# slp-rl/aero

Measured on AMD Instinct MI355X. Metric: real-time-factor (audio-sec/wall-sec), Aero.forward STFT+U-Net+iSTFT, 4->16kHz nfft=512 hop=64 batch=64 per GPU, higher is better.
Workload: dtype f16; 1 GPU; batch=64 synthetic 2s white-noise clips per GPU, 4->16 kHz, aero_4-16_512_64 (nfft=512 hop=64), random-init weights seed 2036, inference, inputs resident in HBM; global_batch=64, clip_samples=8000, frames=501, parallelism=clips sharded over 1 GPU(s), no data-path collective, precision=fp16 operands/storage, fp32 accumulate; STFT/iSTFT/statistics fp32

## Files before the change

aero_amd/_lib.py:

```python
import ctypes as C
import os

_HERE = os.path.dirname(os.path.abspath(__file__))
DEFAULT_LIB = os.path.join(_HERE, 'libaero_hip.so')

ACT_NONE, ACT_RELU, ACT_GELU, ACT_GLU, ACT_SNAKE = 0, 1, 2, 3, 4

i32, i64, vp, fp, dp = C.c_int32, C.c_int64, C.c_void_p, C.c_void_p, C.c_void_p


class ConvDesc(C.Structure):
    _fields_ = [('src0', vp), ('s0_b', i64), ('s0_f', i64), ('s0_t', i64), ('C0', i32),
                ('src1', vp), ('s1_b', i64), ('s1_f', i64), ('s1_t', i64), ('C1', i32),
                ('weight', vp), ('bias', fp),
                ('dst', vp), ('d_b', i64), ('d_f', i64), ('d_t', i64),
                ('dst_f32', i32), ('dst_f_off', i32), ('dst_F', i32),
                ('B', i32), ('Fin', i32), ('Fout', i32), ('T', i32), ('M', i32),
                ('transposed', i32), ('fstride', i32),
                ('ntaps', i32), ('df', i32 * 9), ('dt', i32 * 9),
                ('act', i32),
                ('res', vp), ('r_b', i64), ('r_f', i64), ('r_t', i64),
                ('post_add', fp), ('batch_scale', fp), ('batch_shift', fp),
                ('stats', dp), ('stat_count', C.c_double),
                ('stat_mode', i32), ('stat_G', i32), ('stat_per_row', i32), ('stat_eps', C.c_float),
# ... 88 lines not shown
                ('B', i32), ('F', i32), ('T', i32), ('C', i32)]


class FtbFirstDesc(C.Structure):
    _fields_ = [('xn', vp), ('u', vp), ('gate', vp), ('w2a', vp),
                ('p0', fp), ('p1', fp), ('pb', fp), ('rs', fp), ('a_re', fp), ('a_im', fp), ('bias', fp),
                ('dst', vp), ('B', i32), ('F', i32), ('T', i32), ('C', i32)]


class Enc0Desc(C.Structure):
    _fields_ = [('xn', vp), ('u', vp), ('g', vp), ('rs', fp), ('a_re', fp), ('a_im', fp), ('bias_f', fp),
                ('wc', vp), ('bias_c', fp), ('dst', vp),
                ('B', i32), ('F', i32), ('T', i32), ('C', i32), ('M', i32), ('Fo', i32), ('ktaps', i32), ('stride', i32),
                ('pad', i32), ('act', i32)]


class SeanetConvDesc(C.Structure):
    _fields_ = [('x', vp), ('wimg', vp), ('bias', fp), ('add', vp), ('y', vp),
                ('B', i32), ('Tin', i32), ('Cin', i32), ('Tq', i32), ('M', i32), ('K', i32), ('stride', i32), ('dil', i32), ('pad', i32),
                ('reflect', i32), ('ksteps', i32), ('R', i32), ('P', i32), ('Tout', i32), ('Cout', i32), ('act', i32), ('in_slope', C.c_float)]


class SeanetResDesc(C.Structure):
    _fields_ = [('x', vp), ('w1', vp), ('w2s', vp), ('b1', fp), ('b2s', fp), ('add', vp), ('y', vp),
                ('B', i32), ('T', i32), ('C', i32), ('d', i32), ('ks1', i32), ('ks2', i32), ('slope', C.c_float)]


DCONV_MAX_DEPTH = 4


class DconvLayer(C.Structure):
    _fields_ = [('w1', vp), ('w2', vp), ('consts', fp), ('snake_a', fp),
                ('dilation', i32), ('norm1', i32), ('norm2', i32), ('reserved', i32)]


class DconvDesc(C.Structure):
    _fields_ = [('x', vp), ('y', vp), ('R', i32), ('T', i32), ('C', i32), ('hidden', i32), ('depth', i32), ('act', i32),
                ('F', i32), ('eps', C.c_float), ('layer', DconvLayer * DCONV_MAX_DEPTH)]


class DconvRewriteDesc(C.Structure):
    _fields_ = [('dconv', DconvDesc), ('rw_w', vp), ('rw_bias', fp), ('post_add', fp),
                ('dst', vp), ('d_b', i64), ('d_f', i64), ('d_t', i64)]


_PROTOS = {
    'aero_version': (C.c_char_p, []),
    'aero_last_error': (C.c_char_p, []),
    'aero_last_kernel_name': (C.c_char_p, []),
    'aero_stft_fwd': (i32, [fp, i32, i32, i32, i32, i32, fp, i32, fp, i32, dp, i32, vp]),
    'aero_stft_dft_table_bytes': (i64, [i32]),
    'aero_stft_dft_table': (i32, [fp, i32, i32, vp, vp]),
    'aero_stft_dft_fwd': (i32, [fp, i32, i32, i32, i32, i32, i32, vp, fp, i32, dp, i32, vp]),
    'aero_stft_dft_norm_fwd': (i32, [fp, i32, i32, i32, i32, i32, i32, vp, i32, dp, i32, vp, fp, vp]),
    'aero_spec_normalize': (i32, [fp, i32, i64, dp, vp, fp, vp]),
    'aero_istft_fwd': (i32, [fp, i32, i32, i32, i32, i32, fp, fp, fp, i32, vp]),
    'aero_istft_pitch': (i32, [i32, i32, i32, C.POINTER(i32), C.POINTER(i32)]),
    'aero_istft_pitched_fwd': (i32, [fp, i32, i32, i32, i32, i32, i32, i32, fp, fp, fp, i32, vp]),
    'aero_conv_fwd': (i32, [C.POINTER(ConvDesc), vp]),
    'aero_split_finish': (i32, [fp, i32, fp, i32, vp, i64, i32, vp]),
    'aero_adam_step': (i32, [fp, fp, fp, fp, i64, C.c_float, C.c_float, C.c_float, C.c_float, i32, C.c_float, vp]),
    'aero_adam_step_dev': (i32, [fp, fp, fp, fp, i64, C.c_float, C.c_float, C.c_float, C.c_float, fp, C.c_float, vp]),
    'aero_conv_wgrad': (i32, [C.POINTER(WgradDesc), vp]),
    'aero_conv_wgrad_chunks': (i32, [i32, i32, i32, i32, i32]),
    'aero_norm_bwd_reduce': (i32, [C.POINTER(NormBwdDesc), vp]),
    'aero_norm_bwd_apply': (i32, [C.POINTER(NormBwdDesc), vp]),
    'aero_istft_bwd_prep': (i32, [fp, fp, fp, i32, i32, i32, i32, i32, vp]),
    'aero_istft_bwd_pack': (i32, [fp, fp, i32, i32, i32, i32, i32, vp]),
    'aero_conv_tile_m': (i32, [i32]),
    'aero_conv_ring_bm': (i32, [i32, i32]),
    'aero_convtr_tail_finish': (i32, [fp, fp, fp, fp, fp, fp, i32, i32, i32, i32, i32, vp]),
    'aero_convtr_tail_finish_pitched': (i32, [fp, fp, fp, fp, fp, fp, i32, i32, i32, i32, i32, i32, i32, vp]),
    'aero_conv_kernel_name': (i32, [C.POINTER(ConvDesc), C.c_char_p, i32]),
    'aero_norm_stats': (i32, [C.POINTER(NormDesc), vp]),
    'aero_norm_apply': (i32, [C.POINTER(NormDesc), vp]),
    'aero_gram_stats': (i32, [C.POINTER(GramDesc), vp]),
    'aero_lstm_fwd': (i32, [C.POINTER(LstmDesc), vp]),
    'aero_lstm_geometry': (i32, [i32, C.POINTER(i32), C.POINTER(i32)]),
    'aero_lstm_geometry_in': (i32, [i32, i32, C.POINTER(i32)]),
    'aero_localstate_fwd': (i32, [C.POINTER(AttnDesc), vp]),
    'aero_freqfc_fwd': (i32, [C.POINTER(FreqFcDesc), vp]),
    'aero_ftb_first_fwd': (i32, [C.POINTER(FtbFirstDesc), vp]),
    'aero_enc0_fwd': (i32, [C.POINTER(Enc0Desc), vp]),
    'aero_dconv_row_fwd': (i32, [C.POINTER(DconvDesc), vp]),
    'aero_dconv_row_fits': (i32, [i32, i32, i32, i32]),
    'aero_dconv_row_rewrite_fwd': (i32, [C.POINTER(DconvRewriteDesc), vp]),
    'aero_dconv_row_rewrite_fits': (i32, [i32, i32, i32, i32]),
    'aero_lstm_bwd': (i32, [C.POINTER(LstmBwdDesc), vp]),
    'aero_lstm_bwd_k4p': (i32, [i32]),
    'aero_localstate_bwd': (i32, [C.POINTER(AttnBwdDesc), vp]),
    'aero_freqfc_wgrad': (i32, [vp, vp, vp, fp, fp, i32, i32, i32, i32, i32, vp]),
    'aero_ftb_gate_bwd': (i32, [vp, vp, vp, vp, vp, vp, i32, i32, i32, i32, vp]),
    'aero_sum_bt': (i32, [vp, fp, i32, i32, i32, i32, C.c_float, vp]),
    'aero_frames_op': (i32, [vp, vp, i32, i32, i32, i32, i32, i32, i32, vp]),
    'aero_stft_loss_sums': (i32, [fp, fp, i64, C.c_float, dp, i32, dp, vp]),
    'aero_stft_loss_bwd': (i32, [fp, fp, i64, C.c_float, dp, C.c_float, C.c_float, fp, fp, vp]),
    'aero_irfft_frames': (i32, [fp, i32, i32, i32, i32, fp, fp, vp]),
    'aero_stft_adj_fold': (i32, [fp, fp, i32, i32, i32, i32, i32, i32, vp]),
    'aero_add_f16': (i32, [vp, vp, vp, i64, C.c_float, vp]),
    'aero_scale_cast': (i32, [fp, i32, i64, fp, vp, C.c_float, vp, fp, vp]),
    'aero_scale_f32': (i32, [fp, i64, fp, vp]),
    'aero_gather_pack': (i32, [vp, vp, i32, vp, vp, i64, i32, vp]),
    'aero_debug_probe': (i32, [vp, i32, i32, i32, vp, vp]),
    'aero_bn_running_update': (i32, [dp, i32, C.c_double, C.c_float, fp, fp, vp, vp]),
    'aero_gconv1d_mfma_ok': (i32, [i32, i32, i32, i32, i32, i32, i32]),
    'aero_weightnorm_fwd': (i32, [fp, fp, fp, i32, i32, vp]),
    'aero_weightnorm_bwd': (i32, [fp, i64, i64, i64, fp, fp, fp, fp, fp, fp, fp, fp, i32, i32, i32, i32, vp]),
    'aero_gconv1d_wgrad_slabs': (i32, [i32, i32, i32, i32, i32, i32, i32, i32, i32]),
    'aero_rescale_f16': (i32, [vp, fp, vp, fp, i64, vp, C.c_float, vp, fp, vp]),
    'aero_gconv1d_fwd': (i32, [C.POINTER(GconvDesc), vp]),
    'aero_pw_fwd': (i32, [C.POINTER(PwDesc), vp]),
    'aero_comm_unique_id': (i32, [vp]),
    'aero_comm_init': (i32, [i32, i32, vp, C.POINTER(vp)]),
    'aero_allreduce_f32': (i32, [vp, fp, i64, vp]),
    'aero_allgather': (i32, [vp, vp, vp, i64, vp]),
    'aero_comm_destroy': (i32, [vp]),
    'aero_stream_create': (i32, [i32, C.POINTER(C.c_uint32), i32, C.POINTER(vp)]),
    'aero_stream_destroy': (i32, [vp]),
    'aero_pw_rows': (i32, [i32, i32]),
    'aero_pw_ksteps': (i32, [i32]),
    'aero_squeeze_fwd': (i32, [vp, i64, i64, i64, vp, fp, vp, i32, i32, i32, i32, i32, i32, i32, vp]),
    'aero_leaky_relu': (i32, [vp, i64, C.c_float, vp]),
    'aero_avgpool1d': (i32, [vp, vp, i32, i32, vp]),
    'aero_loss_sum': (i32, [vp, vp, i64, C.c_float, i32, dp, i32, dp, C.c_double, vp]),
    'aero_gconv1d_bwd': (i32, [C.POINTER(GconvBwdDesc), vp]),
    'aero_loss_grad': (i32, [vp, vp, i64, C.c_float, C.c_float, i32, vp, fp, vp]),
    'aero_avgpool1d_bwd': (i32, [vp, vp, i32, i32, vp]),
    'aero_mpd_fold': (i32, [fp, i32, i32, i32, vp, vp]),
    'aero_mpd_unfold_add': (i32, [fp, i32, i32, i32, fp, vp]),
    'aero_mpd_conv0_fwd': (i32, [vp, fp, fp, vp, i32, i32, i32, i32, C.c_float, vp]),
    'aero_mpd_conv0_slabs': (i32, [i32, i32]),
    'aero_mpd_conv0_bwd': (i32, [vp, vp, fp, fp, fp, fp, i32, fp, fp, i32, i32, i32, i32, vp]),
    'aero_mpd_act': (i32, [vp, i32, i32, i32, i32, C.c_float, vp]),
    'aero_seanet_stats': (i32, [fp, i32, i32, C.c_float, fp, vp]),
    'aero_seanet_front': (i32, [fp, fp, fp, fp, i32, i32, i32, i32, i32, i32, i32, vp]),
    'aero_seanet_conv_in': (i32, [fp, fp, fp, vp, i32, i32, i32, vp]),
    'aero_seanet_conv': (i32, [C.POINTER(SeanetConvDesc), vp]),
    'aero_seanet_resblock': (i32, [C.POINTER(SeanetResDesc), vp]),
    'aero_seanet_conv_out': (i32, [vp, vp, fp, fp, fp, fp, i32, i32, i32, i32, C.c_float, vp]),
    'aero_segment_gather': (i32, [vp, i32, vp, vp, i32, vp, vp, i32, i32, fp, vp]),
    'aero_overlap_stitch': (i32, [fp, i32, fp, i32, fp, i32, i32, i64, i32, i32, i32, fp, i64, vp, vp]),
    'aero_wav_finalize': (i32, [fp, vp, i32, i64, fp, vp]),
}

EXPORTS = tuple(_PROTOS)


class AeroHipError(RuntimeError):
    pass


class Lib:

    def __init__(self, path):
        if not os.path.exists(path):
            raise ImportError(
                f'{path} not found: build the gfx950 kernels first (python -c "import __graft_entry__ as g; '
                f'g.build()").  aero_amd has no CPU or eager fallback.')
        self.path = path
        self.cdll = C.CDLL(path)
        for name, (res, args) in _PROTOS.items():
            try:
                fn = getattr(self.cdll, name)
            except AttributeError as e:
                raise ImportError(f'{path} does not export {name}') from e
            fn.restype = res
# ... 34 lines not shown
```

aero_amd/csrc/aero_hip.hip:

```cpp
#include "aero_common.h"
#ifdef AERO_PART
#define AERO_IN(p) (AERO_PART == (p))
#else
#define AERO_IN(p) 1
#endif
#if AERO_IN(0)
#include "k_attn.h"
#include "k_lstm.h"
#include "k_norm.h"
#include "k_gram.h"
#include "k_optim.h"
#endif
#if AERO_IN(1)
#include "k_stft.h"
#include "k_train.h"
#endif
#if AERO_IN(2)
#include "k_conv.h"
#endif
#if AERO_IN(6)
#include "k_conv_ring.h"
#endif
#if AERO_IN(7)
#include "k_pw.h"
// ... 371 lines not shown
}

int aero_scale_f32(float* x, int64_t n, const float* scale, void* stream) {
    const char* err = "";
    int rc = aero_scale_f32_launch(x, n, scale, (hipStream_t)stream, &err);
    return aero_finish(rc, err);
}

int aero_rescale_f16(const void* a, const float* sa, const void* b, const float* sb, int64_t n, void* amax, float target, void* out,
                     float* scale_out, void* stream) {
    const char* err = "";
    int rc = aero_rescale_f16_launch(a, sa, b, sb, n, (unsigned int*)amax, target, out, scale_out, (hipStream_t)stream, &err);
    return aero_finish(rc, err);
}

#endif

#if AERO_IN(2)

int aero_conv_fwd(const aero_conv_desc* d, void* stream) {
    const char* err = "";
    AeroConvK p;
    AeroConvPlan plan;
    int rc = aero_conv_check(d, &err);
    if (rc == AERO_OK) rc = aero_conv_plan(d, p, plan, &err);
    if (rc == AERO_OK) aero_conv_issue(plan, p, (hipStream_t)stream);
    return aero_finish(rc, err);
}

int aero_conv_tile_m(int32_t M) { return aero_conv_pick_bm(M, (M + 127) / 128 * 128); }

int aero_conv_kernel_name(const aero_conv_desc* d, char* name, int32_t cap) {
    if (!name || cap < 96) return aero_fail(AERO_ERR_ARG, "conv_kernel_name: buffer of >= 96 bytes required");
    const char* err = "";
    name[0] = 0;
    AeroConvK p;
    AeroConvPlan plan;
    int rc = aero_conv_check(d, &err);
    if (rc == AERO_OK) rc = aero_conv_plan(d, p, plan, &err);
    if (rc != AERO_OK) return aero_fail(rc, err);
    aero_conv_plan_name(plan, name);
    return AERO_OK;
}

int aero_split_finish(const float* acc, int32_t nsplit, const float* bias, int32_t act, void* dst, int64_t npos, int32_t M, void* stream) {
    const char* err = "";
    int rc = aero_split_finish_launch(acc, nsplit, bias, act, dst, npos, M, (hipStream_t)stream, &err);
    return aero_finish(rc, err);
}

#endif

#if AERO_IN(3)

int aero_freqfc_fwd(const aero_freqfc_desc* d, void* stream) {
    const char* err = "";
    int rc = aero_freqfc_launch(d, (hipStream_t)stream, &err);
    return aero_finish(rc, err);
}

int aero_dconv_row_fwd(const aero_dconv_desc* d, void* stream) {
    const char* err = "";
    int rc = aero_dconv_launch(d, nullptr, (hipStream_t)stream, &err);
    return aero_finish(rc, err);
}

int aero_dconv_row_fits(int T, int C, int hidden, int max_dilation) { return aero_dconv_row_fits_impl(T, C, hidden, max_dilation); }

int aero_dconv_row_rewrite_fwd(const aero_dconv_rewrite_desc* d, void* stream) {
    const char* err = "";
    if (!d) return aero_fail(AERO_ERR_ARG, "dconv rewrite: null descriptor");
    int rc = aero_dconv_launch(&d->dconv, d, (hipStream_t)stream, &err);
    return aero_finish(rc, err);
}

int aero_dconv_row_rewrite_fits(int T, int C, int hidden, int max_dilation) { return aero_dconv_row_fits_impl(T, C, hidden, max_dilation, true); }

int aero_enc0_fwd(const aero_enc0_desc* d, void* stream) {
    const char* err = "";
    int rc = aero_enc0_launch(d, (hipStream_t)stream, &err);
    return aero_finish(rc, err);
}

int aero_ftb_first_fwd(const aero_ftb_first_desc* d, void* stream) {
    const char* err = "";
    int rc = aero_ftb_first_launch(d, (hipStream_t)stream, &err);
    return aero_finish(rc, err);
}

#endif

#if AERO_IN(4)

int aero_conv_wgrad(const aero_wgrad_desc* d, void* stream) {
    const char* err = "";
    int rc = aero_conv_wgrad_launch(d, (hipStream_t)stream, &err);
    return aero_finish(rc, err);
}

int aero_conv_wgrad_chunks(int32_t M, int32_t C, int32_t ntaps, int32_t nrows, int32_t T) {
    if (M < 1 || C < 1 || ntaps < 1 || nrows < 1 || T < 1) return 1;
    bool big;
    int nchunk, SC;
    aero_wgrad_plan(M, C, ntaps, nrows, T, &big, &nchunk, &SC);
    return nchunk;
}

int aero_norm_bwd_reduce(const aero_norm_bwd_desc* d, void* stream) {
    const char* err = "";
    int rc = aero_norm_bwd_launch(d, 0, (hipStream_t)stream, &err);
    return aero_finish(rc, err);
}

int aero_norm_bwd_apply(const aero_norm_bwd_desc* d, void* stream) {
    const char* err = "";
    int rc = aero_norm_bwd_launch(d, 1, (hipStream_t)stream, &err);
    return aero_finish(rc, err);
}

int aero_istft_bwd_prep(const float* dy, const float* inv_env, float* s, int32_t nsig, int32_t L, int32_t Ls, int32_t off, int32_t env_off, void* stream) {
    const char* err = "";
    int rc = aero_istft_bwd_prep_launch(dy, inv_env, s, nsig, L, Ls, off, env_off, (hipStream_t)stream, &err);
    return aero_finish(rc, err);
}

int aero_istft_bwd_pack(const float* spec, float* dz, int32_t nsig, int32_t nbins, int32_t Tsrc, int32_t T, int32_t t_off, void* stream) {
    const char* err = "";
    int rc = aero_istft_bwd_pack_launch(spec, dz, nsig, nbins, Tsrc, T, t_off, (hipStream_t)stream, &err);
    return aero_finish(rc, err);
}

#endif

#if AERO_IN(4)

int aero_gconv1d_mfma_ok(int32_t Cin, int32_t Cout, int32_t groups, int32_t K, int32_t stride, int32_t pad, int32_t reflect) {
    return aero_gconv4_ok(Cin, Cout, groups, K, stride, pad, reflect);
}

int aero_gconv1d_wgrad_slabs(int32_t B, int32_t Tin, int32_t Cin, int32_t Cout, int32_t groups, int32_t K, int32_t stride, int32_t pad,
                             int32_t reflect) {
    if (B < 1 || Tin < 1) return 0;
    const bool c1 = aero_edge_c1_ok(Cin, Cout, groups, K, stride, pad);
    if (c1 || aero_edge_o1_ok(Cin, Cout, groups, K, stride, pad, reflect)) {
        int nb, per;
        aero_edge_wgrad_plan(c1, B, Tin, &nb, &per);
        return B * nb;
    }
    if (!aero_gconv4_ok(Cin, Cout, groups, K, stride, pad, reflect)) return 0;
    const int Tout = (Tin + 2 * pad - K) / stride + 1;
    if (Tout < 1) return 0;
    int ntile, tpc, nchunk;
    aero_gconv4_wgrad_plan(B, Tout, groups, &ntile, &tpc, &nchunk);
    return B * nchunk;
}

int aero_weightnorm_fwd(const float* v, const float* g, float* w, int32_t Cout, int32_t L, void* stream) {
    if (!v || !g || !w || Cout < 1 || L < 1) return aero_fail(AERO_ERR_ARG, "weightnorm_fwd: bad arguments");
    AERO_LAUNCH(aero_weightnorm_fwd_kernel, dim3((unsigned)Cout), dim3(256), (hipStream_t)stream, v, g, w, L);
    return aero_finish(AERO_OK, "");
}

int aero_weightnorm_bwd(const float* dw, int64_t so, int64_t sc, int64_t sk, const float* v, const float* g, const float* db, const float* inv_scale,
                        const float* gl, float* dg, float* dv, float* dbias, int32_t Cout, int32_t cig, int32_t K, int32_t accumulate, void* stream) {
    const char* err = "";
    int rc = aero_weightnorm_bwd_launch(dw, so, sc, sk, v, g, db, inv_scale, gl, dg, dv, dbias, Cout, cig, K, accumulate, (hipStream_t)stream, &err);
// ... 295 lines not shown
```

aero_amd/csrc/k_enc0.h:

```cpp
#pragma once
#include "aero_common.h"

static __device__ __forceinline__ h16x8 aero_splat8(h16 v) { return (h16x8){v, v, v, v, v, v, v, v}; }

struct AeroEnc0K {
    aero_enc0_desc d;
    int Cp, Mpad, Ktot;
};

template <int MFC, int KT, int ROWS>
__global__ __launch_bounds__(256, 2) void aero_enc0_kernel(AeroEnc0K p) {
    constexpr int BN = 128;
    constexpr int BMC = MFC * 16;
    constexpr int CS = BMC + 8;
    h16* Ws = (h16*)AERO_DYN_SMEM;
    const aero_enc0_desc& d = p.d;
    const int nrows = (ROWS - 1) * d.stride + d.ktaps;
    h16* Cs = Ws + d.ktaps * KT * BMC * 32;
    float* cst = (float*)(Cs + BN * CS);
    const int tid = threadIdx.x, lane = tid & 63, wave = aero_uniform(tid >> 6);
    const int g = lane >> 4, col = lane & 15;
    const int C = d.C, T = d.T, M = d.M;
    const int ntt = (T + BN - 1) / BN;
    const int nfb = (d.Fo + ROWS - 1) / ROWS;
    int id = aero_xcd_swizzle((int)blockIdx.x, (int)gridDim.x);
    const int tt = id % ntt;
    id /= ntt;
    const int fb = id % nfb;
    const int b = id / nfb;
    const int fo0 = fb * ROWS, t0 = tt * BN;
    for (int v = tid; v < d.ktaps * KT * BMC * 4; v += 256) {
        const int tile = v / (BMC * 4), rem = v - tile * (BMC * 4);
        const int r = rem >> 2, q = rem & 3;
        const int tap = tile / KT, kt = tile - tap * KT;
        *(h16x8*)&Ws[tile * BMC * 32 + aero_tile_off(r, q)] =
            *(const h16x8*)((const h16*)d.wc + (int64_t)r * p.Ktot + tap * p.Cp + kt * 32 + q * 8);
    }
    if (tid < 64) {
        const bool in = tid < C;
        cst[tid] = in ? d.a_re[tid] : 0.f;
        cst[64 + tid] = in ? d.a_im[tid] : 0.f;
        cst[128 + tid] = in ? d.bias_f[tid] : 0.f;
        cst[192 + tid] = (tid < M && d.bias_c) ? d.bias_c[tid] : 0.f;
        const int fr = fo0 * d.stride - d.pad + tid;
        cst[256 + tid] = (tid < nrows && fr >= 0 && fr < d.F) ? d.rs[fr] : 0.f;
    }
    const int fi_lo = fo0 * d.stride - d.pad;
    h16x8 G[3][2][KT];
    int pos[2];
#pragma unroll
    for (int n = 0; n < 2; ++n) {
        pos[n] = t0 + (wave * 2 + n) * 16 + col;
        const int tq = pos[n] < T ? pos[n] : T - 1;
        const h16* gp = (const h16*)d.g + ((int64_t)b * T + tq) * (3 * C);
#pragma unroll
        for (int q = 0; q < 3; ++q)
#pragma unroll
            for (int ks = 0; ks < KT; ++ks) {
                const int c = ks * 32 + g * 8;
                G[q][n][ks] = c < C ? *(const h16x8*)(gp + q * C + c) : (h16x8){0, 0, 0, 0, 0, 0, 0, 0};
            }
    }
    f32x4 acc[ROWS][MFC][2];
    __syncthreads();
    h16x8 K8[3][KT];
#pragma unroll
    for (int q = 0; q < 3; ++q)
#pragma unroll
        for (int ks = 0; ks < KT; ++ks)
#pragma unroll
            for (int e = 0; e < 8; ++e) K8[q][ks][e] = (h16)cst[q * 64 + ks * 32 + g * 8 + e];
#pragma unroll
    for (int r = 0; r < ROWS; ++r)
#pragma unroll
        for (int i = 0; i < MFC; ++i) {
            acc[r][i][0] = (f32x4){0.f, 0.f, 0.f, 0.f};
            acc[r][i][1] = (f32x4){0.f, 0.f, 0.f, 0.f};
        }
    const h16* xnb = (const h16*)d.xn + (int64_t)b * d.F * T * 2;
    const h16* ub = (const h16*)d.u + (int64_t)b * d.F * T * 2;
    auto load_s = [&](int fi, h16x2 (&uu)[2], h16x2 (&vv)[2]) {
#pragma unroll
        for (int n = 0; n < 2; ++n) {
            uu[n] = (h16x2){0, 0};
            vv[n] = (h16x2){0, 0};
            if (fi >= 0 && fi < d.F && pos[n] < T) {
                uu[n] = *(const h16x2*)(ub + ((int64_t)fi * T + pos[n]) * 2);
                vv[n] = *(const h16x2*)(xnb + ((int64_t)fi * T + pos[n]) * 2);
            }
        }
    };
    h16x2 un[2], vn[2];
    load_s(fi_lo, un, vn);
#pragma unroll 1
    for (int ri = 0; ri < nrows; ++ri) {
        const int fi = fi_lo + ri;
        h16x2 uu[2], vv[2];
#pragma unroll
        for (int n = 0; n < 2; ++n) { uu[n] = un[n]; vv[n] = vn[n]; }
        if (ri + 1 < nrows) load_s(fi + 1, un, vn);
        if (fi < 0 || fi >= d.F) continue;
        const h16 rsf = (h16)cst[256 + ri];
        h16x8 xb[KT][2];
#pragma unroll
        for (int n = 0; n < 2; ++n) {
            const h16x8 ur = aero_splat8(uu[n][0]), ui = aero_splat8(uu[n][1]), re = aero_splat8(vv[n][0]), im = aero_splat8(vv[n][1]);
            const h16x8 rs8 = aero_splat8(rsf);
#pragma unroll
            for (int ks = 0; ks < KT; ++ks) {
                const h16x8 v = G[0][n][ks] * ur + (G[1][n][ks] * ui + (G[2][n][ks] * rs8 + (K8[0][ks] * re + (K8[1][ks] * im + K8[2][ks]))));
                xb[ks][n] = __builtin_elementwise_max(v, (h16x8){0, 0, 0, 0, 0, 0, 0, 0});
            }
        }
#pragma unroll
        for (int r = 0; r < ROWS; ++r) {
            const int j = ri - r * d.stride;
            if (j < 0 || j >= d.ktaps) continue;
            const h16* Wj = Ws + j * KT * BMC * 32;
#pragma unroll
            for (int ks = 0; ks < KT; ++ks)
#pragma unroll
                for (int i = 0; i < MFC; ++i) {
                    const h16x8 a = *(const h16x8*)&Wj[ks * BMC * 32 + aero_tile_off(i * 16 + col, g)];
                    acc[r][i][0] = __builtin_amdgcn_mfma_f32_16x16x32_f16(a, xb[ks][0], acc[r][i][0], 0, 0, 0);
                    acc[r][i][1] = __builtin_amdgcn_mfma_f32_16x16x32_f16(a, xb[ks][1], acc[r][i][1], 0, 0, 0);
                }
        }
    }
    constexpr int nvec = BMC / 8;
#pragma unroll
    for (int r = 0; r < ROWS; ++r) {
        const int fo = fo0 + r;
        if (fo >= d.Fo) break;
#pragma unroll
        for (int i = 0; i < MFC; ++i) {
            const int m = i * 16 + g * 4;
            const f32x4 bc = *(const f32x4*)&cst[192 + m];
#pragma unroll
            for (int n = 0; n < 2; ++n) {
                const int pl = (wave * 2 + n) * 16 + col;
                const f32x4 v = acc[r][i][n] + bc;
                f32x2 lo = {v[0], v[1]}, hi = {v[2], v[3]};
                if (d.act == AERO_ACT_GELU) { lo = aero_gelu2(lo); hi = aero_gelu2(hi); }
                else if (d.act == AERO_ACT_RELU) { lo = {fmaxf(lo[0], 0.f), fmaxf(lo[1], 0.f)}; hi = {fmaxf(hi[0], 0.f), fmaxf(hi[1], 0.f)}; }
                *(h16x4*)&Cs[pl * CS + m] = (h16x4){(h16)lo[0], (h16)lo[1], (h16)hi[0], (h16)hi[1]};
            }
        }
        aero_lds_barrier();
        h16* drow = (h16*)d.dst + (((int64_t)b * d.Fo + fo) * T) * M;
        for (int idx = tid; idx < BN * nvec; idx += 256) {
            const int pl = idx / nvec, cv = idx - pl * nvec;
            const int t = t0 + pl;
            if (t < T) *(h16x8*)(drow + (int64_t)t * M + cv * 8) = *(const h16x8*)&Cs[pl * CS + cv * 8];
        }
        aero_lds_barrier();
    }
}

static int aero_enc0_launch(const aero_enc0_desc* d, hipStream_t stream, const char** err) {
    if (!d || !d->xn || !d->u || !d->g || !d->rs || !d->a_re || !d->a_im || !d->bias_f || !d->wc || !d->dst) { *err = "enc0: null pointer"; return AERO_ERR_ARG; }
    if (d->B < 1 || d->F < 1 || d->T < 1 || d->Fo < 1 || d->ktaps < 1 || d->ktaps > 9 || d->stride < 1 || d->pad < 0) { *err = "enc0: bad geometry"; return AERO_ERR_ARG; }
    if (d->C % 8 || d->C < 8 || d->C > 64) { *err = "enc0: C must be a multiple of 8 in [8,64]"; return AERO_ERR_UNSUPPORTED; }
    if (d->M % 16 || d->M < 16 || d->M > 64) { *err = "enc0: M must be a multiple of 16 in [16,64]"; return AERO_ERR_UNSUPPORTED; }
    if (d->act != AERO_ACT_NONE && d->act != AERO_ACT_RELU && d->act != AERO_ACT_GELU) { *err = "enc0: unsupported act"; return AERO_ERR_UNSUPPORTED; }
    if (d->Fo != (d->F + 2 * d->pad - d->ktaps) / d->stride + 1) { *err = "enc0: Fo inconsistent with F/stride/pad"; return AERO_ERR_ARG; }
    if ((((uintptr_t)d->g | (uintptr_t)d->wc | (uintptr_t)d->dst) & 15) || (((uintptr_t)d->xn | (uintptr_t)d->u) & 3)) { *err = "enc0: unaligned pointer"; return AERO_ERR_ARG; }
    constexpr int ROWS = 4;
    AeroEnc0K p;
    p.d = *d;
    p.Cp = (d->C + 31) / 32 * 32;
    p.Mpad = (d->M + 127) / 128 * 128;
    p.Ktot = d->ktaps * p.Cp;
    const long nwg = (long)d->B * ((d->Fo + ROWS - 1) / ROWS) * ((d->T + 127) / 128);
    if (nwg > 0x7fffffffL) { *err = "enc0: grid too large"; return AERO_ERR_ARG; }
    const int kt = p.Cp / 32, mfc = d->M / 16;
    const int nrows = (ROWS - 1) * d->stride + d->ktaps;
    if (nrows > 64) { *err = "enc0: stride / taps too large"; return AERO_ERR_UNSUPPORTED; }
    const size_t lds = ((size_t)d->ktaps * kt * mfc * 16 * 32 + 128 * (mfc * 16 + 8)) * sizeof(h16) + 320 * sizeof(float);
    if (lds > 160 * 1024) { *err = "enc0: LDS"; return AERO_ERR_UNSUPPORTED; }
    dim3 grid((unsigned)nwg), block(256);
#define AERO_ENC0_GO(MFC_, KT_) AERO_LAUNCH_DYN((aero_enc0_kernel<MFC_, KT_, ROWS>), grid, block, lds, stream, p)
    if (kt == 1) {
        if (mfc == 1) AERO_ENC0_GO(1, 1); else if (mfc == 2) AERO_ENC0_GO(2, 1); else if (mfc == 3) AERO_ENC0_GO(3, 1); else AERO_ENC0_GO(4, 1);
    } else {
        if (mfc == 1) AERO_ENC0_GO(1, 2); else if (mfc == 2) AERO_ENC0_GO(2, 2); else if (mfc == 3) AERO_ENC0_GO(3, 2); else AERO_ENC0_GO(4, 2);
    }
#undef AERO_ENC0_GO
    return AERO_OK;
}
```

include/aero_hip.h:

```cpp
#ifndef AERO_HIP_H
#define AERO_HIP_H
#include <stdint.h>

#ifdef __cplusplus
extern "C" {
#endif

#define AERO_OK 0
#define AERO_ERR_ARG (-1)
#define AERO_ERR_LAUNCH (-2)
#define AERO_ERR_UNSUPPORTED (-3)

enum { AERO_ACT_NONE = 0, AERO_ACT_RELU = 1, AERO_ACT_GELU = 2, AERO_ACT_GLU = 3, AERO_ACT_SNAKE = 4 };

const char* aero_version(void);
const char* aero_last_error(void);
const char* aero_last_kernel_name(void);

int aero_stft_fwd(const float* x, int32_t nsig, int32_t L, int32_t Lp, int32_t n_fft, int32_t hop,
                  const float* window, int32_t n_bins, float* spec, int32_t T, double* stats,
                  int32_t sig_per_item, void* stream);

int64_t aero_stft_dft_table_bytes(int32_t n_fft);
int aero_stft_dft_table(const float* window, int32_t n_fft, int32_t win_off, void* table, void* stream);
// ... 45 lines not shown
int aero_conv_kernel_name(const aero_conv_desc* d, char* name, int32_t cap);

typedef struct {
    const void* src; int64_t s_b, s_f, s_t;
    int32_t B, F, T, C, G, per_row;
    float eps;
    double* stats; double stat_count;
    const float* gamma; const float* beta;
    int32_t act;
    const float* snake_a;
    const float* layer_scale;
    const void* res; int64_t r_b, r_f, r_t;
    void* dst; int64_t d_b, d_f, d_t;
} aero_norm_desc;
int aero_norm_stats(const aero_norm_desc* d, void* stream);
int aero_norm_apply(const aero_norm_desc* d, void* stream);

typedef struct aero_gram_desc {
    const void* x; int64_t s_b, s_f, s_t;
    int32_t B, F, T, C;
    const double* G; const double* g1;
    double* stats;
} aero_gram_desc;
int aero_gram_stats(const aero_gram_desc* d, void* stream);

typedef struct aero_pw_desc {
    const void* x; int64_t x_b, x_f, x_t; int32_t C;
    const void* wimg; const float* bias;
    const double* stats; double stat_count; float stat_eps;
    const float* gamma; const float* beta; const float* layer_scale;
    const float* post_add;
    const void* res; int64_t r_b, r_f, r_t;
    void* dst; int64_t d_b, d_f, d_t;
    int32_t B, F, T, M, act;
    const void* x1; int64_t x1_b, x1_f, x1_t; int32_t C0;
} aero_pw_desc;
int aero_pw_fwd(const aero_pw_desc* d, void* stream);
int aero_squeeze_fwd(const void* x, int64_t x_b, int64_t x_f, int64_t x_t, const void* wimg, const float* bias, void* dst, int32_t B, int32_t F,
                     int32_t T, int32_t C, int32_t M, int32_t rp, int32_t act, void* stream);
int aero_pw_rows(int32_t C, int32_t M);
int aero_pw_ksteps(int32_t C);

typedef struct {
    const void* xproj; const void* xbias; const void* whh; void* out;
    int32_t H, nseq, W, in_mode, out_mode, nframes, S, T;
    const void* x; const void* wih; const float* bias;
    int32_t in_ch, x_pitch;
    void* save_gates; float* save_c;
    int32_t frame_major;
} aero_lstm_desc;
int aero_lstm_fwd(const aero_lstm_desc* d, void* stream);
int aero_lstm_geometry(int32_t H, int32_t* MP, int32_t* KP);
int aero_lstm_geometry_in(int32_t H, int32_t in_ch, int32_t* KPI);

typedef struct {
    const void* qkvd; int64_t ld; void* out;
    int32_t R, T, C, heads, ndecay;
} aero_attn_desc;
int aero_localstate_fwd(const aero_attn_desc* d, void* stream);

typedef struct {
    const void* x; const void* w; const void* gate; void* dst;
    int32_t B, F, T, C;
} aero_freqfc_desc;
int aero_freqfc_fwd(const aero_freqfc_desc* d, void* stream);

typedef struct {
    const void* xn; const void* u; const void* gate; const void* w2a;
    const float* p0; const float* p1; const float* pb; const float* rs;
    const float* a_re; const float* a_im; const float* bias;
    void* dst;
    int32_t B, F, T, C;
} aero_ftb_first_desc;
int aero_ftb_first_fwd(const aero_ftb_first_desc* d, void* stream);

typedef struct {
    const void* xn; const void* u; const void* g;
    const float* rs; const float* a_re; const float* a_im; const float* bias_f;
    const void* wc; const float* bias_c;
    void* dst;
    int32_t B, F, T, C, M, Fo, ktaps, stride, pad, act;
} aero_enc0_desc;
int aero_enc0_fwd(const aero_enc0_desc* d, void* stream);

#define AERO_DCONV_MAX_DEPTH 4
typedef struct {
    const void* w1; const void* w2; const float* consts; const float* snake_a;
    int32_t dilation, norm1, norm2, reserved;
} aero_dconv_layer;
typedef struct {
    const void* x; void* y;
    int32_t R, T, C, hidden, depth, act, F;
    float eps;
    aero_dconv_layer layer[AERO_DCONV_MAX_DEPTH];
} aero_dconv_desc;
int aero_dconv_row_fwd(const aero_dconv_desc* d, void* stream);
int aero_dconv_row_fits(int T, int C, int hidden, int max_dilation);

typedef struct {
    aero_dconv_desc dconv;
    const void* rw_w; const float* rw_bias; const float* post_add;
    void* dst; int64_t d_b, d_f, d_t;
} aero_dconv_rewrite_desc;
int aero_dconv_row_rewrite_fwd(const aero_dconv_rewrite_desc* d, void* stream);
int aero_dconv_row_rewrite_fits(int T, int C, int hidden, int max_dilation);

int aero_adam_step(float* p, const float* g, float* m, float* v, int64_t n, float lr, float beta1, float beta2, float eps,
                   int32_t step, float grad_scale, void* stream);
int aero_adam_step_dev(float* p, const float* g, float* m, float* v, int64_t n, float lr, float beta1, float beta2, float eps,
                       const float* bc, float grad_scale, void* stream);


typedef struct {
    const void* dy; int64_t dy_b, dy_f, dy_t;
    const void* x; int64_t x_b, x_f, x_t;
    float* dw; float* db;
    int32_t B, Fin, Fout, T, M, C, ntaps, fstride;
    int32_t df[9], dt[9];
    float* slabs; int32_t nslab;
    int32_t store, dw_layout, dw_rowlen, dw_coff;
} aero_wgrad_desc;
int aero_conv_wgrad(const aero_wgrad_desc* d, void* stream);
int aero_conv_wgrad_chunks(int32_t M, int32_t C, int32_t ntaps, int32_t nrows, int32_t T);

typedef struct {
    const void* x; int64_t x_b, x_f, x_t;
    const void* dy; int64_t dy_b, dy_f, dy_t;
    void* dx; int64_t dx_b, dx_f, dx_t;
    int32_t B, F, T, C, G, per_row;
    float eps;
    const double* stats; double stat_count;
    const float* gamma; const float* beta; const float* layer_scale;
    int32_t act;
    double* sums;
    float* dgamma; float* dbeta; float* dlayer_scale;
    const float* snake_a; float* dsnake_a;
    double* psums;
} aero_norm_bwd_desc;
int aero_norm_bwd_reduce(const aero_norm_bwd_desc* d, void* stream);
int aero_norm_bwd_apply(const aero_norm_bwd_desc* d, void* stream);

int aero_istft_bwd_prep(const float* dy, const float* inv_env, float* s, int32_t nsig, int32_t L, int32_t Ls, int32_t off, int32_t env_off, void* stream);
int aero_istft_bwd_pack(const float* spec, float* dz, int32_t nsig, int32_t nbins, int32_t Tsrc, int32_t T, int32_t t_off, void* stream);


typedef struct {
    const void* dout; const void* whh_t; const void* save_gates; const float* save_c; void* da;
    int32_t H, nseq, W, out_mode, nframes, S, T;
} aero_lstm_bwd_desc;
int aero_lstm_bwd(const aero_lstm_bwd_desc* d, void* stream);
int aero_lstm_bwd_k4p(int32_t H);

typedef struct {
    const void* qkvd; int64_t ld; const void* out; const void* dout; void* dqkvd; float* qstats;
    int32_t R, T, C, heads, ndecay;
    float decay_scale;
} aero_attn_bwd_desc;
int aero_localstate_bwd(const aero_attn_bwd_desc* d, void* stream);

int aero_freqfc_wgrad(const void* dfc, const void* x, const void* gate, float* dw, float* slabs, int32_t nslab, int32_t B, int32_t F,
                      int32_t T, int32_t C, void* stream);
int aero_ftb_gate_bwd(const void* v, const void* x, const void* gate, const void* add, void* dx, void* dgate, int32_t B, int32_t F,
                      int32_t T, int32_t C, void* stream);

int aero_sum_bt(const void* x, float* out, int32_t B, int32_t F, int32_t T, int32_t C, float scale, void* stream);

// ... 115 lines not shown
```

Measured before the change: 15290 audio-sec/wall-sec.

## Add rolling-segment enc0 kernel reusing overlapping input rows across output rows

Adds a new fused first-encoder kernel used when ktaps equals twice the stride. Each workgroup walks a segment of output frequency rows and computes each input row group once, feeding it into both the current and the previous output row's accumulators. This avoids recomputing the gated input for overlapping taps, which the old kernel redid for every output row. Segment length is picked from the CU count so the grid still fills the device. It is on by default and can be turned off with an environment variable. It costs double-buffered accumulators and LDS, and may lower occupancy for the largest configurations.

```diff
diff --git a/aero_amd/_lib.py b/aero_amd/_lib.py
--- a/aero_amd/_lib.py
+++ b/aero_amd/_lib.py
@@ -194,6 +194,7 @@
     'aero_freqfc_fwd': (i32, [C.POINTER(FreqFcDesc), vp]),
     'aero_ftb_first_fwd': (i32, [C.POINTER(FtbFirstDesc), vp]),
     'aero_enc0_fwd': (i32, [C.POINTER(Enc0Desc), vp]),
+    'aero_enc0_seg_rows': (i32, [i32, i32, i32, i32]),
     'aero_dconv_row_fwd': (i32, [C.POINTER(DconvDesc), vp]),
     'aero_dconv_row_fits': (i32, [i32, i32, i32, i32]),
     'aero_dconv_row_rewrite_fwd': (i32, [C.POINTER(DconvRewriteDesc), vp]),
diff --git a/aero_amd/csrc/aero_hip.hip b/aero_amd/csrc/aero_hip.hip
--- a/aero_amd/csrc/aero_hip.hip
+++ b/aero_amd/csrc/aero_hip.hip
@@ -477,6 +477,8 @@
     return aero_finish(rc, err);
 }
 
+int aero_enc0_seg_rows(int B, int Fo, int ntt, int n_cu) { return aero_enc0_seg_rows_impl(B, Fo, ntt, n_cu > 0 ? n_cu : aero_enc0_n_cu()); }
+
 int aero_ftb_first_fwd(const aero_ftb_first_desc* d, void* stream) {
     const char* err = "";
     int rc = aero_ftb_first_launch(d, (hipStream_t)stream, &err);
diff --git a/aero_amd/csrc/k_enc0.h b/aero_amd/csrc/k_enc0.h
--- a/aero_amd/csrc/k_enc0.h
+++ b/aero_amd/csrc/k_enc0.h
@@ -1,7 +1,15 @@
 #pragma once
+#include <stdlib.h>
 #include "aero_common.h"
 
 static __device__ __forceinline__ h16x8 aero_splat8(h16 v) { return (h16x8){v, v, v, v, v, v, v, v}; }
+static __device__ __forceinline__ h16x2 aero_sel2(bool hi, h16x2 a, h16x2 b) {
+    uint32_t x = hi ? __builtin_bit_cast(uint32_t, b) : __builtin_bit_cast(uint32_t, a);
+#ifndef AERO_EMU
+    asm("" : "+v"(x));
+#endif
+    return __builtin_bit_cast(h16x2, x);
+}
 
 struct AeroEnc0K {
     aero_enc0_desc d;
@@ -157,6 +165,244 @@
     }
 }
 
+struct AeroEnc0RollK {
+    aero_enc0_desc d;
+    int Cp, Ktot, rseg;
+};
+
+static inline int aero_enc0_seg_rows_impl(int B, int Fo, int ntt, int n_cu) {
+    for (int rseg = 64; rseg > 4; rseg >>= 1)
+        if ((int64_t)B * ((Fo + rseg - 1) / rseg) * ntt >= 2 * (int64_t)n_cu) return rseg;
+    return 4;
+}
+
+static inline int aero_enc0_n_cu() {
+#ifdef AERO_EMU
+    return 2;
+#else
+    static int n_cu = 0;
+    if (n_cu <= 0) {
+        int dev = 0, v = 0;
+        if (hipGetDevice(&dev) != hipSuccess || hipDeviceGetAttribute(&v, hipDeviceAttributeMultiprocessorCount, dev) != hipSuccess || v < 1) v = 256;
+        n_cu = v;
+    }
+    return n_cu;
+#endif
+}
+
+template <int MFC, int C8, int HP>
+__global__ __launch_bounds__(256, (MFC == 4 && C8 >= 6 && HP == 2) ? 1 : 2) void aero_enc0_roll_kernel(AeroEnc0RollK p) {
+    constexpr int BN = 128;
+    constexpr int BMC = MFC * 16;
+    constexpr int CS = BMC + 8;
+    constexpr int C = C8 * 8;
+    constexpr int KS = C8 / 2;
+    constexpr int NG = C8 == 6 ? 3 : C8 == 8 ? 2 : 1;
+    constexpr int STRIDE = 2 * HP, NTP = 2 * HP;
+    h16* Ws = (h16*)AERO_DYN_SMEM;
+    h16* Cs = Ws + NTP * KS * BMC * 32;
+    float* cst = (float*)(Cs + 2 * BN * CS);
+    const aero_enc0_desc& d = p.d;
+    const int tid = threadIdx.x, lane = tid & 63, wave = aero_uniform(tid >> 6);
+    const int g = lane >> 4, col = lane & 15;
+    const int T = d.T;
+    const int ntt = (T + BN - 1) / BN;
+    const int nseg = (d.Fo + p.rseg - 1) / p.rseg;
+    int id = aero_xcd_swizzle((int)blockIdx.x, (int)gridDim.x);
+    const int tt = id % ntt;
+    id /= ntt;
+    const int sg = id % nseg;
+    const int b = id / nseg;
+    const int fo0 = sg * p.rseg, t0 = tt * BN;
+    const int nr = d.Fo - fo0 < p.rseg ? d.Fo - fo0 : p.rseg;
+    const int fi_lo = fo0 * STRIDE - d.pad;
+    for (int v = tid; v < NTP * KS * BMC * 4; v += 256) {
+        const int tile = v / (BMC * 4), rem = v - tile * (BMC * 4);
+        const int r = rem >> 2, q = rem & 3;
+        const int tp = tile / KS, s = tile - tp * KS;
+        const int o = 4 * s + q;
+        *(h16x8*)&Ws[tile * BMC * 32 + aero_tile_off(r, q)] =
+            *(const h16x8*)((const h16*)d.wc + (int64_t)r * p.Ktot + (2 * tp + o / C8) * p.Cp + (o % C8) * 8);
+    }
+    if (tid < 64) {
+        const bool in = tid < C;
+        cst[tid] = in ? d.a_re[tid] : 0.f;
+        cst[64 + tid] = in ? d.a_im[tid] : 0.f;
+        cst[128 + tid] = in ? d.bias_f[tid] : 0.f;
+        cst[192 + tid] = (tid < d.M && d.bias_c) ? d.bias_c[tid] : 0.f;
+    }
+    for (int i = tid; i < (nr + 1) * STRIDE; i += 256) {
+        const int fr = fi_lo + i;
+        cst[256 + i] = (fr >= 0 && fr < d.F) ? d.rs[fr] : 0.f;
+    }
+    h16x8 G[3][2][NG];
+    int pos[2];
+#pragma unroll
+    for (int n = 0; n < 2; ++n) {
+        pos[n] = t0 + (wave * 2 + n) * 16 + col;
+        pos[n] = pos[n] < T ? pos[n] : T - 1;
+        const h16* gp = (const h16*)d.g + ((int64_t)b * T + pos[n]) * (3 * C);
+#pragma unroll
+        for (int q = 0; q < 3; ++q)
+#pragma unroll
+            for (int sl = 0; sl < NG; ++sl) G[q][n][sl] = *(const h16x8*)(gp + q * C + ((4 * sl + g) % C8) * 8);
+    }
+    f32x4 accA[MFC][2], accB[MFC][2];
+    __syncthreads();
+    h16x8 K8[3][NG];
+#pragma unroll
+    for (int q = 0; q < 3; ++q)
+#pragma unroll
+        for (int sl = 0; sl < NG; ++sl)
+#pragma unroll
+            for (int e = 0; e < 8; ++e) K8[q][sl][e] = (h16)cst[q * 64 + ((4 * sl + g) % C8) * 8 + e];
+#pragma unroll
+    for (int i = 0; i < MFC; ++i) {
+        accA[i][0] = accA[i][1] = (f32x4){0.f, 0.f, 0.f, 0.f};
+        accB[i][0] = accB[i][1] = (f32x4){0.f, 0.f, 0.f, 0.f};
+    }
+    const h16* xnb = (const h16*)d.xn + (int64_t)b * d.F * T * 2;
+    const h16* ub = (const h16*)d.u + (int64_t)b * d.F * T * 2;
+    const uint32_t poff[2] = {(uint32_t)pos[0] * 4u, (uint32_t)pos[1] * 4u};
+    auto load_s = [&](int pg, h16x2 (&su)[STRIDE][2], h16x2 (&sv)[STRIDE][2]) {
+#pragma unroll
+        for (int j = 0; j < STRIDE; ++j) {
+            int fi = fi_lo + pg * STRIDE + j;
+            fi = fi < 0 ? 0 : fi >= d.F ? d.F - 1 : fi;
+            const char* ur = (const char*)(ub + (int64_t)fi * T * 2);
+            const char* vr = (const char*)(xnb + (int64_t)fi * T * 2);
+#pragma unroll
+            for (int n = 0; n < 2; ++n) {
+                su[j][n] = *(const h16x2*)(ur + poff[n]);
+                sv[j][n] = *(const h16x2*)(vr + poff[n]);
+            }
+        }
+    };
+    auto group = [&](int pg, f32x4 (&aN)[MFC][2], f32x4 (&aO)[MFC][2], const h16x2 (&su)[STRIDE][2], const h16x2 (&sv)[STRIDE][2]) {
+        const bool do_new = pg < nr, do_old = pg >= 1;
+#pragma unroll
+        for (int q = 0; q < HP; ++q) {
+            const int fi0 = fi_lo + pg * STRIDE + 2 * q;
+            const bool v0 = fi0 >= 0 && fi0 < d.F, v1 = fi0 + 1 >= 0 && fi0 + 1 < d.F;
+            if (!(v0 || v1)) continue;
+            const f32x2 rsp = *(const f32x2*)&cst[256 + pg * STRIDE + 2 * q];
+            const h16 rs0 = (h16)rsp[0], rs1 = (h16)rsp[1];
+            h16x8 xb[KS][2];
+#pragma unroll
+            for (int s = 0; s < KS; ++s) {
+                const bool mixed = (4 * s) / C8 != (4 * s + 3) / C8;
+                const bool hi = mixed ? (4 * s + g >= C8) : ((4 * s) / C8 == 1);
+                const int sl = s % NG;
+                const h16x8 rs8 = aero_splat8(hi ? rs1 : rs0);
+                const h16x8 kb = (hi ? v1 : v0) ? K8[2][sl] : aero_splat8((h16)-65504.f);
+#pragma unroll
+                for (int n = 0; n < 2; ++n) {
+                    const h16x2 uu = mixed ? aero_sel2(hi, su[2 * q][n], su[2 * q + 1][n]) : su[2 * q + (hi ? 1 : 0)][n];
+                    const h16x2 vv = mixed ? aero_sel2(hi, sv[2 * q][n], sv[2 * q + 1][n]) : sv[2 * q + (hi ? 1 : 0)][n];
+                    const h16x8 ur = aero_splat8(uu[0]), ui = aero_splat8(uu[1]), re = aero_splat8(vv[0]), im = aero_splat8(vv[1]);
+                    const h16x8 v = G[0][n][sl] * ur + (G[1][n][sl] * ui + (G[2][n][sl] * rs8 + (K8[0][sl] * re + (K8[1][sl] * im + kb))));
+                    xb[s][n] = __builtin_elementwise_max(v, (h16x8){0, 0, 0, 0, 0, 0, 0, 0});
+                }
+            }
+            if (do_new) {
+                const h16* Wj = Ws + q * KS * BMC * 32;
+#pragma unroll
+                for (int s = 0; s < KS; ++s)
+#pragma unroll
+                    for (int i = 0; i < MFC; ++i) {
+                        const h16x8 a = *(const h16x8*)&Wj[s * BMC * 32 + aero_tile_off(i * 16 + col, g)];
+                        aN[i][0] = __builtin_amdgcn_mfma_f32_16x16x32_f16(a, xb[s][0], aN[i][0], 0, 0, 0);
+                        aN[i][1] = __builtin_amdgcn_mfma_f32_16x16x32_f16(a, xb[s][1], aN[i][1], 0, 0, 0);
+                    }
+            }
+            if (do_old) {
+                const h16* Wj = Ws + (HP + q) * KS * BMC * 32;
+#pragma unroll
+                for (int s = 0; s < KS; ++s)
+#pragma unroll
+                    for (int i = 0; i < MFC; ++i) {
+                        const h16x8 a = *(const h16x8*)&Wj[s * BMC * 32 + aero_tile_off(i * 16 + col, g)];
+                        aO[i][0] = __builtin_amdgcn_mfma_f32_16x16x32_f16(a, xb[s][0], aO[i][0], 0, 0, 0);
+                        aO[i][1] = __builtin_amdgcn_mfma_f32_16x16x32_f16(a, xb[s][1], aO[i][1], 0, 0, 0);
+                    }
+            }
+        }
+    };
+    constexpr int nvec = BMC / 8;
+    auto emit = [&](f32x4 (&acc)[MFC][2], int fo, h16* Cb) {
+#pragma unroll
+        for (int i = 0; i < MFC; ++i) {
+            const int m = i * 16 + g * 4;
+            const f32x4 bc = *(const f32x4*)&cst[192 + m];
+#pragma unroll
+            for (int n = 0; n < 2; ++n) {
+                const int pl = (wave * 2 + n) * 16 + col;
+                const f32x4 v = acc[i][n] + bc;
+                f32x2 lo = {v[0], v[1]}, hi = {v[2], v[3]};
+                if (d.act == AERO_ACT_GELU) { lo = aero_gelu2(lo); hi = aero_gelu2(hi); }
+                else if (d.act == AERO_ACT_RELU) { lo = {fmaxf(lo[0], 0.f), fmaxf(lo[1], 0.f)}; hi = {fmaxf(hi[0], 0.f), fmaxf(hi[1], 0.f)}; }
+                *(h16x4*)&Cb[pl * CS + m] = (h16x4){(h16)lo[0], (h16)lo[1], (h16)hi[0], (h16)hi[1]};
+                acc[i][n] = (f32x4){0.f, 0.f, 0.f, 0.f};
+            }
+        }
+        aero_lds_barrier();
+        h16* drow = (h16*)d.dst + (((int64_t)b * d.Fo + fo) * T) * BMC;
+        for (int idx = tid; idx < BN * nvec; idx += 256) {
+            const int pl = idx / nvec, cv = idx - pl * nvec;
+            const int t = t0 + pl;
+            if (t < T) *(h16x8*)(drow + (int64_t)t * BMC + cv * 8) = *(const h16x8*)&Cb[pl * CS + cv * 8];
+        }
+    };
+    h16x2 Su0[STRIDE][2], Sv0[STRIDE][2], Su1[STRIDE][2], Sv1[STRIDE][2];
+    load_s(0, Su0, Sv0);
+#pragma unroll 1
+    for (int pg = 0; pg <= nr; pg += 2) {
+        load_s(pg + 1, Su1, Sv1);
+        group(pg, accA, accB, Su0, Sv0);
+        if (pg >= 1) emit(accB, fo0 + pg - 1, Cs + BN * CS);
+        if (pg + 1 > nr) break;
+        load_s(pg + 2, Su0, Sv0);
+        group(pg + 1, accB, accA, Su1, Sv1);
+        emit(accA, fo0 + pg, Cs);
+    }
+}
+
+static int aero_enc0_roll_on() {
+    static const int on = [] { const char* e = getenv("AERO_ENC0_ROLL"); return (e && e[0] == '0') ? 0 : 1; }();
+    return on;
+}
+
+static int aero_enc0_roll_launch(const aero_enc0_desc* d, hipStream_t stream, const char** err) {
+    AeroEnc0RollK p;
+    p.d = *d;
+    p.Cp = (d->C + 31) / 32 * 32;
+    p.Ktot = d->ktaps * p.Cp;
+    const int ntt = (d->T + 127) / 128;
+    p.rseg = aero_enc0_seg_rows_impl(d->B, d->Fo, ntt, aero_enc0_n_cu());
+    const long nwg = (long)d->B * ((d->Fo + p.rseg - 1) / p.rseg) * ntt;
+    if (nwg > 0x7fffffffL) { *err = "enc0: grid too large"; return AERO_ERR_ARG; }
+    const int mfc = d->M / 16, c8 = d->C / 8, hp = d->stride / 2;
+    const size_t lds = ((size_t)d->ktaps * d->C * mfc * 16 + 2 * 128 * (mfc * 16 + 8)) * sizeof(h16) + (256 + 65 * 4 + 4) * sizeof(float);
+    if (lds > 160 * 1024) { *err = "enc0: LDS"; return AERO_ERR_UNSUPPORTED; }
+    dim3 grid((unsigned)nwg), block(256);
+#define AERO_ENC0_ROLL_GO(MFC_, C8_, HP_) AERO_LAUNCH_DYN((aero_enc0_roll_kernel<MFC_, C8_, HP_>), grid, block, lds, stream, p)
+#define AERO_ENC0_ROLL_M(C8_, HP_)                                                                                        \
+    do {                                                                                                                  \
+        if (mfc == 1) AERO_ENC0_ROLL_GO(1, C8_, HP_); else if (mfc == 2) AERO_ENC0_ROLL_GO(2, C8_, HP_);                  \
+        else if (mfc == 3) AERO_ENC0_ROLL_GO(3, C8_, HP_); else AERO_ENC0_ROLL_GO(4, C8_, HP_);                           \
+    } while (0)
+#define AERO_ENC0_ROLL_C(HP_)                                                                                             \
+    do {                                                                                                                  \
+        if (c8 == 2) AERO_ENC0_ROLL_M(2, HP_); else if (c8 == 4) AERO_ENC0_ROLL_M(4, HP_);                                \
+        else if (c8 == 6) AERO_ENC0_ROLL_M(6, HP_); else AERO_ENC0_ROLL_M(8, HP_);                                        \
+    } while (0)
+    if (hp == 1) AERO_ENC0_ROLL_C(1); else AERO_ENC0_ROLL_C(2);
+#undef AERO_ENC0_ROLL_C
+#undef AERO_ENC0_ROLL_M
+#undef AERO_ENC0_ROLL_GO
+    return AERO_OK;
+}
+
 static int aero_enc0_launch(const aero_enc0_desc* d, hipStream_t stream, const char** err) {
     if (!d || !d->xn || !d->u || !d->g || !d->rs || !d->a_re || !d->a_im || !d->bias_f || !d->wc || !d->dst) { *err = "enc0: null pointer"; return AERO_ERR_ARG; }
     if (d->B < 1 || d->F < 1 || d->T < 1 || d->Fo < 1 || d->ktaps < 1 || d->ktaps > 9 || d->stride < 1 || d->pad < 0) { *err = "enc0: bad geometry"; return AERO_ERR_ARG; }
@@ -165,6 +411,7 @@
     if (d->act != AERO_ACT_NONE && d->act != AERO_ACT_RELU && d->act != AERO_ACT_GELU) { *err = "enc0: unsupported act"; return AERO_ERR_UNSUPPORTED; }
     if (d->Fo != (d->F + 2 * d->pad - d->ktaps) / d->stride + 1) { *err = "enc0: Fo inconsistent with F/stride/pad"; return AERO_ERR_ARG; }
     if ((((uintptr_t)d->g | (uintptr_t)d->wc | (uintptr_t)d->dst) & 15) || (((uintptr_t)d->xn | (uintptr_t)d->u) & 3)) { *err = "enc0: unaligned pointer"; return AERO_ERR_ARG; }
+    if (aero_enc0_roll_on() && d->ktaps == 2 * d->stride && d->stride % 2 == 0 && d->C % 16 == 0) return aero_enc0_roll_launch(d, stream, err);
     constexpr int ROWS = 4;
     AeroEnc0K p;
     p.d = *d;
diff --git a/include/aero_hip.h b/include/aero_hip.h
--- a/include/aero_hip.h
+++ b/include/aero_hip.h
@@ -151,6 +151,7 @@
     int32_t B, F, T, C, M, Fo, ktaps, stride, pad, act;
 } aero_enc0_desc;
 int aero_enc0_fwd(const aero_enc0_desc* d, void* stream);
+int aero_enc0_seg_rows(int B, int Fo, int ntt, int n_cu);
 
 #define AERO_DCONV_MAX_DEPTH 4
 typedef struct {
```

Result: no change. 15410 audio-sec/wall-sec (median of 6 runs) (+0.8%).
